# alexandervakhitov/lld-slam

Hardware: NVIDIA B200
Metric: local_ba_lm_iters_per_sec (higher is better)
Workload: dtype f64

## Files before the change

### lld_slam_b200/csrc/ba.cu

```cuda
#include <algorithm>
#include <atomic>
#include <chrono>
#include <condition_variable>
#include <functional>
#include <mutex>
#include <thread>
#include <cstdlib>
#include <cstring>
#ifdef __linux__
#include <sched.h>
#endif
#include <numeric>
#include <vector>

#include "ba_kernels.cuh"
#include "cr_solver.cuh"
#include "sp_solver.cuh"
#include "lld_ctx.h"

#include <array>
#include <map>
#include <string>

#ifdef LLD_WITH_NCCL
// ... 922 lines not shown
          spos[i] = oi;
          mask[oi] = (uint32_t)key[i];
          run += __builtin_popcountll(key[i]);
          w0[oi + 1] = run;
        }
      });
    };
    slots(p->pt_off, pt_order, pt_key, pt_spos, pts_mask, pts_w0, pl_off);
    slots(p->ln_off, ln_order, ln_key, ln_spos, lns_mask, lns_w0, ll_off);
    n_pw = (size_t)pts_w0[n_pt]; n_lw = (size_t)lns_w0[n_ln];
    stage("dense: W slots");
    int PIECE_CAP = 128;
    while (PIECE_CAP > 8 && (long long)(n_pt + n_ln) * 5 / (2 * PIECE_CAP) < 16LL * c->sm_count) PIECE_CAP >>= 1;
    using Job = BaDenseJob;
    auto& jobs = H.jobs;
    if (jobs.size() < 2 * (size_t)nw) jobs.resize(2 * (size_t)nw);
    for (size_t j = 0; j < 2 * (size_t)nw; j++) jobs[j].clear();
    const size_t n_jobs = 2 * (size_t)nw;
    par_for(2 * nw, [&](int jid) {
      const int kind = jid / nw, w = jid % nw;
      Job& J = jobs[jid];
      const int* loff = kind == 0 ? p->pt_off : p->ln_off;
      const pvec<uint32_t>& mask = kind == 0 ? pts_mask : lns_mask;
      const int g0 = w_g0[w];
      int b = loff[w];
      while (b < loff[w + 1]) {
        int e = b + 1;
        while (e < loff[w + 1] && mask[e] == mask[b] && e - b < PIECE_CAP) e++;
        const uint32_t m = mask[b];
        const int n = __builtin_popcount(m);
        if (n > 0) {
          const int pc = (int)J.pb.size();
          J.pb.push_back(b); J.pe.push_back(e); J.pn.push_back(n); J.pout.push_back(J.dsize);
          const int npair = n * (n + 1) / 2, ntask = 6 * npair + n;
          int hl[32], k = 0;
          for (int h = 0; h < 32; h++)
            if ((m >> h) & 1u) hl[k++] = h;
          int pr = 0;
          for (int ia = 0; ia < n; ia++)
            for (int ib = ia; ib < n; ib++, pr++) J.gb.push_back({nb_off[g0 + hl[ia]] + (hl[ib] - hl[ia]), J.dsize + 36LL * pr});
          for (int ia = 0; ia < n; ia++) J.gv.push_back({g0 + hl[ia], J.dsize + 36LL * npair + (long long)SCHUR_KS * ia});
          for (int t0 = 0; t0 < 2 * npair + n; t0 += SP_TPB) { J.itp.push_back(pc); J.itt.push_back(t0); }
          J.dsize += 36LL * npair + (long long)SCHUR_KS * n;
        }
        b = e;
      }
    });
    stage("dense: pieces");
    std::vector<long long> jd(n_jobs + 1, 0);
    std::vector<int> ji(n_jobs + 1, 0);
    for (size_t jid = 0; jid < n_jobs; jid++) {
      jd[jid + 1] = jd[jid] + jobs[jid].dsize;
      ji[jid + 1] = ji[jid] + (int)jobs[jid].itp.size();
    }
    dpart_total = jd[n_jobs];
    n_items_pt = ji[std::min<size_t>((size_t)nw, n_jobs)];
    n_items_all = ji[n_jobs];
    H.it_rec.resize(std::max(ji[n_jobs], 1));
    gb_off.assign(nb_g.size() + 1, 0);
    gv_off.assign(nG + 1, 0);
    par_for((int)n_jobs, [&](int jid) {
      Job& J = jobs[jid];
      const int ibase = ji[jid];
      const int kind = jid / nw, jw = jid % nw;
      for (size_t k = 0; k < J.itp.size(); k++) {
        const int q = J.itp[k];
        SchurItem& R = H.it_rec[ibase + k];
        R.l0 = J.pb[q]; R.nl = J.pe[q] - J.pb[q]; R.n = J.pn[q]; R.t0 = J.itt[k];
        R.w = jw; R.w0 = (kind == 0 ? pts_w0 : lns_w0)[J.pb[q]]; R.out = J.pout[q] + jd[jid];
        schur_item_shape(kind == 0 ? 3 : 4, R.n, R.nl, R.t0, &R.lc, &R.S, &R.nchunk);
      }
    });
    stage("dense: item records");
    {
      auto& tmp = H.it_tmp; auto& keys = H.it_keys;
      tmp.resize(H.it_rec.size()); keys.resize(H.it_rec.size());
      auto item_order = [&](int kind) {
        const int i0 = kind == 0 ? 0 : n_items_pt, i1 = kind == 0 ? n_items_pt : ji[n_jobs];
        const int cntk = i1 - i0;
        if (cntk <= 0) return;
        const int G = std::min(cntk, 4 * c->sm_count);
        constexpr int NB = 1024;
        std::vector<int> cnt(NB + 1, 0);
        for (int i = i0; i < i1; i++) {
          const SchurItem& R = H.it_rec[i];
          const int ntask = R.n * (R.n + 1) + R.n;
          const uint64_t cost = 64 + (uint64_t)R.nl * (uint64_t)(std::min(ntask - R.t0, (int)SP_TPB) + R.n + 1);
          const int bkt = NB - 1 - (int)std::min<uint64_t>(cost >> 5, NB - 1);
          keys[i] = (uint64_t)bkt;
          cnt[bkt + 1]++;
          tmp[i] = R;
        }
        for (int q = 0; q < NB; q++) cnt[q + 1] += cnt[q];
        for (int i = i0; i < i1; i++) {
          const int k = cnt[(int)keys[i]]++;
          const int r = k / G, j = k - r * G, len = std::min(G, cntk - r * G);
          const int pos = (r & 1) ? len - 1 - j : j;
          H.it_rec[i0 + r * G + pos] = tmp[i];
        }
      };
      par_for(nw + 2, [&](int t) {
        if (t < 2) { item_order(t); return; }
        const int w = t - 2;
        for (int kind = 0; kind < 2; kind++) {
          Job& J = jobs[(size_t)kind * nw + w];
          for (auto& x : J.gb) gb_off[x.first + 1]++;
          for (auto& x : J.gv) gv_off[x.first + 1]++;
        }
      });
    }
    stage("dense: item order + gather counts");
    for (size_t i = 0; i < nb_g.size(); i++) gb_off[i + 1] += gb_off[i];
    for (int i = 0; i < nG; i++) gv_off[i + 1] += gv_off[i];
    gb_src.resize(std::max<size_t>((size_t)gb_off[nb_g.size()], 1));
    gv_src.resize(std::max<size_t>((size_t)gv_off[nG], 1));
    {
      std::vector<int> curb(gb_off.begin(), gb_off.end() - 1), curv(gv_off.begin(), gv_off.end() - 1);
      par_for(nw, [&](int w) {
        for (int kind = 0; kind < 2; kind++) {
          const size_t jid = (size_t)kind * nw + w;
// ... 145 lines not shown
      return LLD_ERR_UNSUPPORTED;
    }
  }
  std::vector<long long> w_scr(nw, 0);
  long long scr_total = 0;
  for (int w = 0; w < nw; w++) {
    const long long n = 6LL * (w_g0[w + 1] - w_g0[w]);
    w_scr[w] = scr_total;
    if (S->max_n > SMEM_SOLVE_MAX_N && !v.env_mode) scr_total += n * n + 8 * n + 40;
  }

  stage("chunks");
  UP(tmp_i, kf_win.data(), n_kf); v.kf_win = tmp_i;
  int *d_pt_win, *d_ln_win, *d_pe_pt, *d_lc_ln, *d_pe_wpos, *d_lc_wpos;
  DEV(d_pt_win, int, n_pt); v.pt_win = d_pt_win;
  DEV(d_ln_win, int, n_ln); v.ln_win = d_ln_win;
  UP(tmp_i, kf_g.data(), n_kf); v.kf_g = tmp_i;
  UP(tmp_i, g_kf.data(), nG); v.g_kf = tmp_i;
  UP(tmp_i, w_g0.data(), nw + 1); v.w_g0 = tmp_i;
  DEV(d_pe_pt, int, n_pe); v.pe_pt = d_pe_pt;
  DEV(d_lc_ln, int, n_lc); v.lc_ln = d_lc_ln;
  UP(tmp_i, pe_pos.data(), dense ? 0 : n_pe); v.pe_pos = tmp_i;
  UP(tmp_i, lc_pos.data(), dense ? 0 : n_lc); v.lc_pos = tmp_i;
  UP(tmp_i, ch_g.data(), n_ch); v.ch_g = tmp_i;
  UP(tmp_i, ch_begin.data(), n_ch); v.ch_begin = tmp_i;
  UP(tmp_i, ch_end.data(), n_ch); v.ch_end = tmp_i;
  UP(tmp_i, ch_seg0.data(), ch_seg0.size()); v.ch_seg0 = tmp_i;
  UP(tmp_i, seg_begin.data(), seg_begin.size()); v.seg_begin = tmp_i;
  UP(tmp_i, seg_end.data(), seg_end.size()); v.seg_end = tmp_i;
  UP(tmp_i, g_chp0.data(), nG + 1); v.g_chp0 = tmp_i;
  UP(tmp_i, g_chl0.data(), nG + 1); v.g_chl0 = tmp_i;
  UP(tmp_i, nb_off.data(), nG + 1); v.nb_off = tmp_i;
  UP(tmp_i, nb_g.data(), nb_g.size()); v.nb_g = tmp_i;
  int *d_pl_tab = nullptr, *d_ll_tab = nullptr;
  DEV(d_pl_tab, int, std::max(pl_tab_total, 1LL)); v.pl_tab = d_pl_tab;
  DEV(d_ll_tab, int, std::max(ll_tab_total, 1LL)); v.ll_tab = d_ll_tab;
  long long* tmp_l;
  UP(tmp_l, pl_tab_off.data(), nG); v.pl_tab_off = tmp_l;
  UP(tmp_l, ll_tab_off.data(), nG); v.ll_tab_off = tmp_l;
  UP(tmp_l, ch_S_off.data(), n_ch); v.ch_S_off = tmp_l;
  UP(tmp_i, pt_spos.data(), n_pt); v.pt_spos = tmp_i;
  UP(tmp_i, ln_spos.data(), n_ln); v.ln_spos = tmp_i;
  UP(tmp_i, pts_w0.data(), n_pt + 1); v.pts_w0 = tmp_i;
  UP(tmp_i, lns_w0.data(), n_ln + 1); v.lns_w0 = tmp_i;
  DEV(d_pe_wpos, int, n_pe); v.pe_wpos = d_pe_wpos;
  DEV(d_lc_wpos, int, n_lc); v.lc_wpos = d_lc_wpos;
  { SchurItem* tmp_r; UP(tmp_r, H.it_rec.data(), (size_t)n_items_all); v.it_rec = tmp_r; }
  UP(tmp_i, gb_off.data(), gb_off.size()); v.gb_off = tmp_i;
  UP(tmp_l, gb_src.data(), gb_src.size()); v.gb_src = tmp_l;
  UP(tmp_i, gv_off.data(), gv_off.size()); v.gv_off = tmp_i;
  UP(tmp_l, gv_src.data(), gv_src.size()); v.gv_src = tmp_l;
  {
    uint32_t* tmp_m;
    UP(tmp_m, pts_mask.data(), n_pt); v.pts_mask = tmp_m;
    UP(tmp_m, lns_mask.data(), n_ln); v.lns_mask = tmp_m;
  }
  UP(tmp_l, w_scr.data(), nw); v.w_scratch_off = tmp_l;
  UP(tmp_i, env_first.data(), env_first.size()); v.env_first = tmp_i;
  UP(tmp_i, env_blk_last.data(), env_blk_last.size()); v.env_blk_last = tmp_i;
  UP(tmp_l, env_rowptr.data(), env_rowptr.size()); v.env_rowptr = tmp_l;

  stage("H2D enqueue");
  if (c->host_only) return LLD_OK;
  for (int b = 0; b < 2; b++) {
    DEV(v.pose_qt[b], double, 7 * (size_t)n_kf);
    DEV(v.pose_Rt[b], double, 12 * (size_t)n_kf);
// ... 67 lines not shown
    const bool dense_single = v.dense_mode && !(global_mode && c->n_ranks > 1) && v.n_slices == 1 && S->max_n <= SMEM_SOLVE_MAX_N && !v.env_mode;
    S->forked = allow && dense_single;
    S->use_graph = allow && dense_single;
    S->lean = dense_single;
  }
  {
    auto grid = [](int n) { return (n + 255) / 256; };
    if (n_pt) LLD_LAUNCH(c, k_expand_owner, grid(n_pt), 256, 0, n_pt, nw, v.pt_off, d_pt_win);
    if (n_ln) LLD_LAUNCH(c, k_expand_owner, grid(n_ln), 256, 0, n_ln, nw, v.ln_off, d_ln_win);
    if (n_pe) LLD_LAUNCH(c, k_expand_owner, grid(n_pe), 256, 0, n_pe, n_pt, v.pt_obs_off, d_pe_pt);
    if (n_lc) LLD_LAUNCH(c, k_expand_owner, grid(n_lc), 256, 0, n_lc, n_ln, v.ln_obs_off, d_lc_ln);
    if (!v.dense_mode) {
      LLD_CUDA(c, cudaMemsetAsync(d_pl_tab, 0xFF, sizeof(int) * (size_t)std::max(pl_tab_total, 1LL), c->stream));
      LLD_CUDA(c, cudaMemsetAsync(d_ll_tab, 0xFF, sizeof(int) * (size_t)std::max(ll_tab_total, 1LL), c->stream));
      if (n_plist) LLD_LAUNCH(c, k_build_tab, grid(n_plist), 256, 0, n_plist, nG, v.pl_off, v.pl_edge, v.pt_obs_off, v.pe_pt, v.pe_kf, v.kf_g,
                              v.pe_pos, v.nb_off, v.nb_g, v.pl_tab_off, d_pl_tab);
      if (n_llist) LLD_LAUNCH(c, k_build_tab, grid(n_llist), 256, 0, n_llist, nG, v.ll_off, v.ll_cell, v.ln_obs_off, v.lc_ln, v.lc_kf, v.kf_g,
                              v.lc_pos, v.nb_off, v.nb_g, v.ll_tab_off, d_ll_tab);
      if (tab_check) {
        std::vector<int> back((size_t)std::max(std::max(pl_tab_total, ll_tab_total), 1LL));
        for (int which = 0; which < 2; which++) {
          const long long tot = which ? ll_tab_total : pl_tab_total;
          LLD_CUDA(c, cudaMemcpyAsync(back.data(), which ? d_ll_tab : d_pl_tab, sizeof(int) * (size_t)tot, cudaMemcpyDeviceToHost, c->stream));
          LLD_CUDA(c, cudaStreamSynchronize(c->stream));
          const pvec<int>& ref = which ? ll_tab : pl_tab;
          long long bad = 0;
          for (long long k = 0; k < tot; k++) bad += back[(size_t)k] != ref[(size_t)k];
          fprintf(stderr, "[lld_ba_upload] LLD_TAB_CHECK %s table: %lld entries, %lld differ from the host build\n", which ? "line" : "point", tot, bad);
          if (bad) { snprintf(c->err, sizeof(c->err), "device-built position table differs from the host build"); return LLD_ERR_CUDA; }
        }
      }
    }
    if (v.dense_mode) {
      if (n_pe) LLD_LAUNCH(c, k_dense_wpos, grid(n_pe), 256, 0, n_pe, v.pe_pt, v.pe_kf, v.kf_g, v.pt_win, v.w_g0, v.pt_spos, v.pts_mask, v.pts_w0, d_pe_wpos);
      if (n_lc) LLD_LAUNCH(c, k_dense_wpos, grid(n_lc), 256, 0, n_lc, v.lc_ln, v.lc_kf, v.kf_g, v.ln_win, v.w_g0, v.ln_spos, v.lns_mask, v.lns_w0, d_lc_wpos);
    }
    LLD_CUDA(c, cudaGetLastError());
  }
  if (v.dense_mode) {
    LLD_CUDA(c, lld_raise_dyn_smem(k_schur_tile<3>, (size_t)SP_SMEM_BYTES));
    LLD_CUDA(c, lld_raise_dyn_smem(k_schur_tile<4>, (size_t)SP_SMEM_BYTES));
  }
  if (v.env_mode && S->use_cr) {
    LLD_CUDA(c, lld_raise_dyn_smem(k_cr_factor, sizeof(double) * ((size_t)S->cr.m * S->cr.m + 8 * (size_t)S->cr.m + 40)));
    LLD_CUDA(c, lld_raise_dyn_smem(k_cr_solve<15>, sizeof(double) * ((size_t)S->cr.m * S->cr.m + CR_RPT * CR_TC)));
    LLD_CUDA(c, lld_raise_dyn_smem(k_cr_solve<20>, sizeof(double) * ((size_t)S->cr.m * S->cr.m + CR_RPT * CR_TC)));
  } else if (v.env_mode && S->use_sp) {
    LLD_CUDA(c, lld_raise_dyn_smem(k_sp_factor, sizeof(double) * ((size_t)S->sp.m * S->sp.m + 8 * (size_t)S->sp.m + 40)));
    LLD_CUDA(c, lld_raise_dyn_smem(k_sp_solve<15>, sizeof(double) * ((size_t)S->sp.m * S->sp.m + CR_RPT * CR_TC)));
    LLD_CUDA(c, lld_raise_dyn_smem(k_sp_solve<20>, sizeof(double) * ((size_t)S->sp.m * S->sp.m + CR_RPT * CR_TC)));
  } else if (v.env_mode) LLD_CUDA(c, lld_raise_dyn_smem(k_solve_env, (size_t)(int)S->env_smem));
  else if (S->max_n <= SMEM_SOLVE_MAX_N)
    LLD_CUDA(c, lld_raise_dyn_smem(k_solve<true>, (size_t)(int)(sizeof(double) * ((size_t)S->max_n * S->max_n + 8 * (size_t)S->max_n + 40))));
  S->topo_ok = topo_cache && th != 0;
  return LLD_OK;
}

static inline int cdiv(int a, int b) { return (a + b - 1) / b; }

static int ba_init_state(LldCtx* c) {
  BaState* S = c->ba;
  BaView& v = S->v;
  const int n = std::max({v.n_kf, v.n_pt, v.n_ln, v.n_pe, v.n_lc, v.n_free_total, 1});
  LLD_LAUNCH(c, k_init_state, cdiv(n, 256), 256, 0, v, S->d_kf_Tcw_in, S->d_pt_in, S->d_ln_in, v.lc_right);
  LLD_CUDA(c, cudaGetLastError());
  return LLD_OK;
// ... 249 lines not shown
    if (r) return r;
  } else if (v.env_mode) {
    LLD_LAUNCH(c, k_solve_env, 1, 1024, S->env_smem, v);
  } else if (S->max_n <= SMEM_SOLVE_MAX_N) { int r = launch_solve<true>(c, v, S->max_n); if (r) return r; }
  else { int r = launch_solve<false>(c, v, S->max_n); if (r) return r; }
  if (par) LLD_CUDA(c, cudaEventRecord(c->ev_fork, s0));
  LLD_CUDA(c, fork(s1));
  if (v.n_pt && v.n_pt <= PT_WIDE_MAX) LLD_LAUNCH_S(c, s0, k_backsub_points<4>, cdiv(v.n_pt * 4, LM_TPB), LM_TPB, 0, v);
  else if (v.n_pt) LLD_LAUNCH_S(c, s0, k_backsub_points<1>, gp, LM_TPB, 0, v);
  { int r = launch_line_kernel(c, s1, v, false); if (r) return r; }
  LLD_CUDA(c, join(0));
  if (fused) {
    LLD_LAUNCH(c, k_decide_fused, v.n_win, FUSED_RED_TPB, 0, v, round, stop_now);
  } else {
    LLD_LAUNCH(c, k_reduce_trial, v.n_win * v.n_slices, 256, 0, v);
    LLD_LAUNCH(c, k_sum_trial, cdiv(v.n_win, 64), 64, 0, v);
    if (multi) { int r = ba_allreduce_trial(c); if (r) return r; }
    LLD_LAUNCH(c, k_decide, cdiv(v.n_win, 64), 64, 0, v, round, stop_now);
  }
  LLD_CUDA(c, cudaGetLastError());
  return LLD_OK;
}

static int ba_run_round(LldCtx* c, int maxit, int round, const volatile uint8_t* stop) {
  BaState* S = c->ba;
  BaView& v = S->v;
  LLD_LAUNCH(c, k_round_init, cdiv(v.n_win, 64), 64, 0, v, maxit, round);
  if (maxit <= 0) return LLD_OK;
  int* h_active = reinterpret_cast<int*>(c->pinned);
  const bool multi = S->global_mode && c->n_ranks > 1;
  const int hard_cap = maxit * 10 + 4;
  static const int group_len = getenv("LLD_BA_GROUP") ? std::max(1, atoi(getenv("LLD_BA_GROUP"))) : 2;
  int launched = 0;
  auto one_step = [&](int stop_now) -> int {
    const bool first = launched == 0;
    const int kind = (S->lean && !first) ? 1 : 0;
    if (S->use_graph && !c->prof_on && !stop_now && round < 2) {
      if (!S->graph_fresh[round][kind]) {
        const int64_t l0 = c->launches;
        cudaGraph_t g = nullptr;
        std::lock_guard<std::mutex> lk(lld_capture_mutex());
        LLD_CUDA(c, cudaStreamBeginCapture(c->stream, cudaStreamCaptureModeThreadLocal));
        int r = ba_step(c, round, 0, first);
        cudaError_t e = cudaStreamEndCapture(c->stream, &g);
        if (r) { if (g) cudaGraphDestroy(g); return r; }
        LLD_CUDA(c, e);
        bool updated = false;
        if (c->ba_graph[round][kind]) {
          cudaGraphExecUpdateResultInfo info;
          if (cudaGraphExecUpdate(c->ba_graph[round][kind], g, &info) == cudaSuccess) updated = true;
          else {
            cudaGetLastError();
            cudaGraphExecDestroy(c->ba_graph[round][kind]);
            c->ba_graph[round][kind] = nullptr;
          }
        }
        if (!updated) e = cudaGraphInstantiate(&c->ba_graph[round][kind], g, 0);
        cudaGraphDestroy(g);
        LLD_CUDA(c, e);
        c->ba_graph_kernels[round][kind] = (int)(c->launches - l0);
        c->launches = l0;
        S->graph_fresh[round][kind] = true;
      }
      {
        std::lock_guard<std::mutex> lk(lld_capture_mutex());
        LLD_CUDA(c, cudaGraphLaunch(c->ba_graph[round][kind], c->stream));
      }
      c->launches += c->ba_graph_kernels[round][kind];
      return LLD_OK;
    }
    return ba_step(c, round, stop_now, first);
  };
  for (int k = 0;; k++) {
    const int slot = k & 1;
    if (k >= 2) {
      LLD_CUDA(c, cudaEventSynchronize(c->ev_grp[slot]));
      if (h_active[slot] <= 0) break;
    }
    int stop_now = (stop && *stop) ? 1 : 0;
#ifdef LLD_WITH_NCCL
    if (multi && stop) {
      h_active[2] = stop_now;
      LLD_CUDA(c, cudaMemcpyAsync(v.n_active_win + 1, &h_active[2], sizeof(int), cudaMemcpyHostToDevice, c->stream));
      LLD_NCCL(c, ncclAllReduce(v.n_active_win + 1, v.n_active_win + 1, 1, ncclInt, ncclMax, reinterpret_cast<ncclComm_t>(c->comm), c->stream));
      LLD_CUDA(c, cudaMemcpyAsync(&h_active[2], v.n_active_win + 1, sizeof(int), cudaMemcpyDeviceToHost, c->stream));
      LLD_CUDA(c, cudaStreamSynchronize(c->stream));
      stop_now = h_active[2];
    }
#endif
    const int n = stop_now ? 1 : group_len;
    for (int s2 = 0; s2 < n; s2++) {
      int r = one_step(stop_now);
      if (r) return r;
      launched++;
    }
    LLD_CUDA(c, cudaMemcpyAsync(&h_active[slot], v.n_active_win, sizeof(int), cudaMemcpyDeviceToHost, c->stream));
    LLD_CUDA(c, cudaEventRecord(c->ev_grp[slot], c->stream));
    if (stop_now) break;
    if (launched >= hard_cap + 2 * group_len) {
      LLD_CUDA(c, cudaStreamSynchronize(c->stream));
      snprintf(c->err, sizeof(c->err), "LM step budget exhausted (%d steps, %d windows still active)", launched, h_active[slot]);
      return LLD_ERR_CUDA;
    }
  }
  LLD_CUDA(c, cudaStreamSynchronize(c->stream));
  return LLD_OK;
}

static int ba_download(LldCtx* c, const lld_ba_problem* p, lld_ba_result* out, bool local) {
  BaState* S = c->ba;
  BaView& v = S->v;
  const int n = std::max({v.n_kf, v.n_pt, v.n_ln, 1});
  if (local) {
    if (v.n_pe) LLD_LAUNCH(c, k_flag_points, cdiv(v.n_pe, 256), 256, 0, v, S->d_pt_bad);
    if (v.n_ln) LLD_LAUNCH(c, k_final_lines, cdiv(v.n_ln, 128), 128, 0, v, S->d_ln_bad);
  }
  LLD_LAUNCH(c, k_export, cdiv(n, 256), 256, 0, v, S->d_out_kf, S->d_out_pt, S->d_out_ln, S->d_ln_in);
  LLD_CUDA(c, cudaGetLastError());
  LLD_CUDA(c, cudaEventRecord(c->ev[2], c->stream));
  auto D2H = [&](void* dst, const void* src, size_t bytes) -> cudaError_t {
    if (!dst || !bytes) return cudaSuccess;
    return cudaMemcpyAsync(dst, src, bytes, cudaMemcpyDeviceToHost, c->stream);
  };
  LLD_CUDA(c, D2H(out->kf_Tcw, S->d_out_kf, sizeof(double) * 12 * (size_t)v.n_kf));
  LLD_CUDA(c, D2H(out->pt_xyz, S->d_out_pt, sizeof(double) * 3 * (size_t)v.n_pt));
  LLD_CUDA(c, D2H(out->ln_x0_dir, S->d_out_ln, sizeof(double) * 6 * (size_t)v.n_ln));
  LLD_CUDA(c, D2H(out->pt_obs_bad, S->d_pt_bad, (size_t)v.n_pe));
  LLD_CUDA(c, D2H(out->ln_obs_bad, S->d_ln_bad, 2 * (size_t)v.n_lc));
// ... 319 lines not shown
```

### lld_slam_b200/csrc/ba.cuh

```cuda
#pragma once
#include <stdint.h>

namespace lld {

enum : int { PH_LIN = 0, PH_RETRY = 1, PH_DONE = 2 };

constexpr int SCHUR_KS = 6;

struct BaParams {
  int robust_pt, robust_ln;
  double delta_pt_mono, delta_pt_stereo, delta_ln_mono, delta_ln_stereo;
  double chi2_pt_mono, chi2_pt_stereo;
  int ln_norm;
  int ln_filter;
};

struct __align__(16) SchurItem {
  int l0, nl, n, t0;
  int w, lc;
  long long w0;
  long long out;
  int S, nchunk;
};

struct BaView {
  int n_win, n_kf, n_pt, n_ln, n_pe, n_lc;
  int n_free_total;
  int n_chunks;
  const int *kf_off, *pt_off, *ln_off;
  const int *kf_win, *pt_win, *ln_win;
  const int* kf_g;
  const int* g_kf;
  const int* w_g0;
  const double* kf_intr;
  const double* kf_lcam;
  const int* pt_obs_off;
  const int* pe_kf;
  const int* pe_pt;
  const float* pe_uvr;
  const float* pe_info;
  const int* ln_obs_off;
  const int* lc_kf;
  const int* lc_ln;
  const float* lc_left;
  const float* lc_right;
  const double* lc_info;
  const uint8_t* lc_stereo;
  int n_chunks_pt;
  const int* pl_off;
  const int* pl_edge;
  const int* pe_pos;
  const int* ll_off;
  const int* ll_cell;
  const int* lc_pos;
  const int* ch_g;
  const int* ch_begin;
  const int* ch_end;
  const int* ch_seg0;
  const int* seg_begin;
  const int* seg_end;
  const int* g_chp0;
  const int* g_chl0;
  const int* nb_off;
  const int* nb_g;
  const int* pl_tab;
  const long long* pl_tab_off;
  const int* ll_tab;
  const long long* ll_tab_off;
  int n_fold, n_fold_pt;
  const int* fold_off;
  const int* fold_dst;
  const int* fold_src;
  int dense_mode;
  const int* pt_sorted;
  const int* ln_sorted;
  const int* pt_spos;
  const int* ln_spos;
  const uint32_t* pts_mask;
  const uint32_t* lns_mask;
  const int* pts_w0;
  const int* lns_w0;
  const int* pe_wpos;
  const int* lc_wpos;
  int n_items;
  int n_items_pt;
  const SchurItem* it_rec;
  const int* gb_off;
  const long long* gb_src;
  const int* gv_off;
  const long long* gv_src;
  double* pe_Wl;
  double* lc_Wl;
  double* pts_D;
  double* lns_D;
  double* dpart;
  double* pose_qt[2];
  double* pose_Rt[2];
// ... 66 lines not shown
```

### lld_slam_b200/csrc/ba_kernels.cuh

```cuda
#pragma once
#include <cfloat>
#include <cstdio>

#include "ba.cuh"
#include "lld_math.cuh"

namespace lld {

#define LM_TPB 128

__device__ __forceinline__ double warp_sum(double v) {
#pragma unroll
  for (int o = 16; o > 0; o >>= 1) v += __shfl_down_sync(0xffffffffu, v, o);
  return v;
}
__device__ __forceinline__ double warp_max(double v) {
#pragma unroll
  for (int o = 16; o > 0; o >>= 1) v = fmax(v, __shfl_down_sync(0xffffffffu, v, o));
  return v;
}
__device__ __forceinline__ double block_sum(double v, double* sm ) {
  const int lane = threadIdx.x & 31, wid = threadIdx.x >> 5;
  v = warp_sum(v);
  __syncthreads();
// ... 995 lines not shown
  const double lam = v.w_lambda[w];
  for (int t = threadIdx.x; t < ld; t += blockDim.x) {
    const int j = t / 6, c = t - 6 * j;
    double s[6] = {0, 0, 0, 0, 0, 0};
    double sb = 0;
    for (int rng = 0; rng < 2; rng++) {
      const int c0 = rng == 0 ? v.g_chp0[g] : v.g_chl0[g], c1 = rng == 0 ? v.g_chp0[g + 1] : v.g_chl0[g + 1];
      for (int ch = c0; ch < c1; ch++) {
        const double* part = v.ch_S + v.ch_S_off[ch];
#pragma unroll
        for (int r = 0; r < 6; r++) s[r] += part[(size_t)r * ld + t];
        if (j == 0) sb += part[(size_t)6 * ld + c];
      }
    }
    double* S = v.S_blk + 36 * (size_t)(v.nb_off[g] + j);
#pragma unroll
    for (int r = 0; r < 6; r++) {
      double d = 0.0;
      if (j == 0 && with_diag) {
        const int rr = r < c ? r : c, cc = r < c ? c : r;
        d = v.g_Hpp[21 * (size_t)g + (rr * 6 - (rr * (rr - 1)) / 2 + (cc - rr))];
        if (r == c) d += lam;
      }
      S[6 * r + c] = d - s[r];
    }
    if (j == 0) v.g_bs[6 * (size_t)g + c] = (with_diag ? v.g_bp[6 * (size_t)g + c] : 0.0) - sb;
  }
}

constexpr int SP_TPB = 128;
constexpr int SP_CAP_WD = 2304;
constexpr int SP_CAP_Z = 2560;
constexpr int SP_SMEM_BYTES = (2 * SP_CAP_WD + SP_CAP_Z) * 8;
constexpr int SP_MAX_S = 16;

__device__ __forceinline__ void cp_async16(void* dst_smem, const void* src) {
  const unsigned s = (unsigned)__cvta_generic_to_shared(dst_smem);
  asm volatile("cp.async.cg.shared.global [%0], [%1], 16;\n" ::"r"(s), "l"(src));
}

inline void schur_item_shape(int D, int n, int nl, int t0, int* lc, int* S, int* nchunk) {
  const int WS = 6 * D, DS = D == 3 ? 10 : 14;
  const int ntask = n * (n + 1) + n;
  int ntb = ntask - t0 < SP_TPB ? ntask - t0 : SP_TPB;
  if (ntb < 1) ntb = 1;
  int L = SP_CAP_WD / (n * WS + DS);
  const int Lz = SP_CAP_Z / ((n + 1) * WS);
  if (Lz < L) L = Lz;
  if (nl < L) L = nl;
  int s = SP_TPB / ntb;
  if (s > SP_MAX_S) s = SP_MAX_S;
  if (s > L / 2) s = L / 2;
  if (s < 1) s = 1;
  *lc = L; *S = s; *nchunk = (nl + L - 1) / L;
}

template <int D>
__global__ void __launch_bounds__(SP_TPB, 4) k_schur_tile(BaView v, int item_base, int n_items) {
  constexpr int WS = 6 * D;
  constexpr int DS = D == 3 ? 10 : 14;
  constexpr int OFF_C = D * (D + 1) / 2;
  extern __shared__ __align__(16) double sp_smem[];
  double* const sZ = sp_smem + 2 * SP_CAP_WD;
  const int tid = threadIdx.x, lane = tid & 31;
  const int G = gridDim.x;
  const int cnt = (n_items - (int)blockIdx.x + G - 1) / G;
  const SchurItem* items = v.it_rec + item_base + blockIdx.x;
  const double* Wbase = D == 3 ? v.pe_Wl : v.lc_Wl;
  const double* Dbase = D == 3 ? v.pts_D : v.lns_D;

  int scan_base = -32;
  unsigned scan_mask = 0;
  auto next_item = [&]() -> int {
    while (true) {
      if (scan_mask) {
        const int j = __ffs(scan_mask) - 1;
        scan_mask &= scan_mask - 1;
        return scan_base + j;
      }
      scan_base += 32;
      if (scan_base >= cnt) return -1;
      const int j = scan_base + lane;
      bool a = false;
      if (j < cnt) a = v.w_phase[items[(size_t)j * G].w] != PH_DONE;
      scan_mask = __ballot_sync(0xffffffffu, a);
    }
  };
  auto load_item = [&](int k, SchurItem& R) {
    const int4* p = reinterpret_cast<const int4*>(items + (size_t)k * G);
    const int4 a = p[0], b = p[1];
    R.l0 = a.x; R.nl = a.y; R.n = a.z; R.t0 = a.w;
    R.w = b.x;
    R.w0 = ((long long)(unsigned)b.w << 32) | (unsigned)b.z;
    const int4 c2 = p[2];
    R.out = ((long long)(unsigned)c2.y << 32) | (unsigned)c2.x;
    R.lc = b.y; R.S = c2.z; R.nchunk = c2.w;
  };
  auto issue = [&](const SchurItem& R, int c, int b) {
    const int rowW = R.n * WS;
    const int Lc = R.lc;
    const int lc0 = c * Lc, m = min(Lc, R.nl - lc0);
    double* sW = sp_smem + b * SP_CAP_WD;
    double* sD = sW + Lc * rowW;
    const double* gW = Wbase + (size_t)R.w0 * WS + (size_t)lc0 * rowW;
    const int nW = m * rowW / 2;
    for (int i = tid; i < nW; i += SP_TPB) cp_async16(sW + 2 * i, gW + 2 * i);
    const double* gD = Dbase + (size_t)(R.l0 + lc0) * DS;
    const int nD = m * DS / 2;
    for (int i = tid; i < nD; i += SP_TPB) cp_async16(sD + 2 * i, gD + 2 * i);
  };

  int cur = next_item();
  if (cur < 0) return;
  SchurItem R, Rn;
  load_item(cur, R);
  issue(R, 0, 0);
  asm volatile("cp.async.commit_group;\n" ::);
  int nxt = next_item();
  Rn = R;
  if (nxt >= 0) load_item(nxt, Rn);
  int buf = 0, c = 0;
  while (true) {
    const int n = R.n, nl = R.nl;
    const int npair = n * (n + 1) / 2, ntask = 2 * npair + n;
    const int ntb = min(SP_TPB, ntask - R.t0);
    const int rowW = n * WS, rowZ = (n + 1) * WS;
    const int Lc = R.lc, nchunk = R.nchunk, S = R.S;
    const int s = tid / ntb, tl = tid - s * ntb;
    const bool act = s < S;
    int ia = 0, zb = n, h = 0;
    {
      const int task = R.t0 + tl;
      if (task < 2 * npair) {
        int pr = task >> 1;
        h = task & 1;
        while (pr >= n - ia) { pr -= n - ia; ia++; }
        zb = ia + pr;
      } else {
        ia = min(task - 2 * npair, n - 1);
      }
    }
    const int zl0 = tid / (n + 1), zb0 = tid - zl0 * (n + 1);
    const int zdl = SP_TPB / (n + 1), zdb = SP_TPB - zdl * (n + 1);
    double acc[18];
#pragma unroll
    for (int q = 0; q < 18; q++) acc[q] = 0.0;
    for (c = 0; c < nchunk; c++, buf ^= 1) {
      if (c + 1 < nchunk) issue(R, c + 1, buf ^ 1);
      else if (nxt >= 0) issue(Rn, 0, buf ^ 1);
      asm volatile("cp.async.commit_group;\n" ::);
      asm volatile("cp.async.wait_group 1;\n" ::: "memory");
      __syncthreads();
      const int m = min(Lc, nl - c * Lc);
      const double* sW = sp_smem + buf * SP_CAP_WD;
      const double* sD = sW + Lc * rowW;
      for (int i = tid, l = zl0, b = zb0; i < m * (n + 1); i += SP_TPB) {
        const double* Dv = sD + l * DS;
        double* z = sZ + l * rowZ + b * WS;
        if (b < n) {
          const double* wv = sW + l * rowW + b * WS;
          double dm[D][D];
#pragma unroll
          for (int k = 0; k < D; k++)
#pragma unroll
            for (int j = 0; j < D; j++) {
              const int r = k < j ? k : j, c2 = k < j ? j : k;
              dm[k][j] = Dv[r * D - (r * (r - 1)) / 2 + (c2 - r)];
            }
#pragma unroll
          for (int cc = 0; cc < 6; cc++) {
            double wb[D];
#pragma unroll
            for (int j = 0; j < D; j++) wb[j] = wv[cc * D + j];
#pragma unroll
            for (int k = 0; k < D; k++) {
              double zz = 0;
#pragma unroll
              for (int j = 0; j < D; j++) zz += dm[k][j] * wb[j];
              z[cc * D + k] = zz;
            }
          }
        } else {
#pragma unroll
          for (int k = 0; k < WS; k++) z[k] = k < D ? Dv[OFF_C + k] : 0.0;
        }
        l += zdl; b += zdb;
        if (b > n) { b -= n + 1; l++; }
      }
      __syncthreads();
      if (act) {
        const double* wa_p = sW + ia * WS;
        const double* z_p = sZ + zb * WS + h * 3 * D;
#pragma unroll 2
        for (int l = s; l < m; l += S) {
          double wa[WS];
          const double* wp = wa_p + l * rowW;
#pragma unroll
          for (int k = 0; k < WS; k += 2) {
            const double2 t2 = *reinterpret_cast<const double2*>(wp + k);
            wa[k] = t2.x; wa[k + 1] = t2.y;
          }
          const double* zp = z_p + l * rowZ;
#pragma unroll
          for (int cc = 0; cc < 3; cc++) {
            double z[D];
#pragma unroll
            for (int k = 0; k < D; k++) z[k] = zp[cc * D + k];
#pragma unroll
            for (int r = 0; r < 6; r++) {
              double a2 = acc[cc * 6 + r];
#pragma unroll
              for (int k = 0; k < D; k++) a2 += wa[D * r + k] * z[k];
              acc[cc * 6 + r] = a2;
            }
          }
        }
      }
      __syncthreads();
    }
    double* out = v.dpart + R.out;
    if (S == 1) {
      if (tid < ntb) {
        const int task = R.t0 + tl;
        if (task < 2 * npair) {
          double* o = out + (size_t)(task >> 1) * 36 + (task & 1) * 18;
#pragma unroll
          for (int q = 0; q < 18; q++) o[q] = acc[q];
        } else {
          double* o = out + (size_t)36 * npair + (size_t)(task - 2 * npair) * SCHUR_KS;
#pragma unroll
          for (int q = 0; q < 6; q++) o[q] = acc[q];
        }
      }
    } else {
      double* red = sZ;
      if (act)
#pragma unroll
        for (int q = 0; q < 18; q++) red[(s * ntb + tl) * 18 + q] = acc[q];
      __syncthreads();
      for (int e = tid; e < ntb * 18; e += SP_TPB) {
        const int tl2 = e / 18, q = e - 18 * tl2;
        const int task = R.t0 + tl2;
        size_t o;
        if (task < 2 * npair) o = (size_t)(task >> 1) * 36 + (task & 1) * 18 + q;
        else if (q < 6) o = (size_t)36 * npair + (size_t)(task - 2 * npair) * SCHUR_KS + q;
        else continue;
        double sum = 0;
        for (int s2 = 0; s2 < S; s2++) sum += red[(s2 * ntb + tl2) * 18 + q];
        out[o] = sum;
      }
    }
    if (nxt < 0) break;
    cur = nxt;
    R = Rn;
    nxt = next_item();
    if (nxt >= 0) load_item(nxt, Rn);
  }
}

__global__ void __launch_bounds__(256) k_reduce_piece(BaView v, int n_blocks) {
  const int t = blockIdx.x * blockDim.x + threadIdx.x;
  if (t < n_blocks * 36) {
    const int blk = t / 36, e = t - 36 * blk, c = e / 6, r = e - 6 * c;
    int lo = 0, hi = v.n_free_total;
    while (hi - lo > 1) {
      const int mid = (lo + hi) >> 1;
      if (v.nb_off[mid] <= blk) lo = mid;
      else hi = mid;
    }
    const int g = lo, j = blk - v.nb_off[g];
    const int w = v.kf_win[v.g_kf[g]];
    if (v.w_phase[w] == PH_DONE) return;
    double s = 0;
    const int q1 = v.gb_off[blk + 1];
    int q = v.gb_off[blk];
    for (; q + 8 <= q1; q += 8) {
      long long o[8];
      double a[8];
#pragma unroll
      for (int k = 0; k < 8; k++) o[k] = v.gb_src[q + k];
#pragma unroll
      for (int k = 0; k < 8; k++) a[k] = v.dpart[o[k] + e];
#pragma unroll
      for (int k = 0; k < 8; k++) s += a[k];
    }
    for (; q + 4 <= q1; q += 4) {
      const long long o0 = v.gb_src[q], o1 = v.gb_src[q + 1], o2 = v.gb_src[q + 2], o3 = v.gb_src[q + 3];
      const double a0 = v.dpart[o0 + e], a1 = v.dpart[o1 + e], a2 = v.dpart[o2 + e], a3 = v.dpart[o3 + e];
      s += a0; s += a1; s += a2; s += a3;
    }
    for (; q < q1; q++) s += v.dpart[v.gb_src[q] + e];
    double d = 0.0;
    if (j == 0) {
      const int rr = r < c ? r : c, cc = r < c ? c : r;
      d = v.g_Hpp[21 * (size_t)g + (rr * 6 - (rr * (rr - 1)) / 2 + (cc - rr))];
      if (r == c) d += v.w_lambda[w];
    }
    v.S_blk[36 * (size_t)blk + 6 * r + c] = d - s;
  } else {
    const int u = t - n_blocks * 36;
    const int g = u / 6, r = u - 6 * g;
    if (g >= v.n_free_total) return;
    const int w = v.kf_win[v.g_kf[g]];
    if (v.w_phase[w] == PH_DONE) return;
    double s = 0;
    for (int q = v.gv_off[g]; q < v.gv_off[g + 1]; q++) s += v.dpart[v.gv_src[q] + r];
    v.g_bs[6 * (size_t)g + r] = v.g_bp[6 * (size_t)g + r] - s;
  }
}

__global__ void __launch_bounds__(256) k_reduce_piece_warp(BaView v, int n_blocks) {
  const int wi = blockIdx.x * (blockDim.x >> 5) + (threadIdx.x >> 5);
  const int lane = threadIdx.x & 31;
  if (wi < n_blocks * 6) {
    const int blk = wi / 6, c = wi - 6 * blk;
    int lo = 0, hi = v.n_free_total;
    while (hi - lo > 1) {
      const int mid = (lo + hi) >> 1;
      if (v.nb_off[mid] <= blk) lo = mid;
      else hi = mid;
    }
    const int g = lo, j = blk - v.nb_off[g];
    const int w = v.kf_win[v.g_kf[g]];
    if (v.w_phase[w] == PH_DONE) return;
    double s[6] = {0, 0, 0, 0, 0, 0};
    for (int q = v.gb_off[blk] + lane; q < v.gb_off[blk + 1]; q += 32) {
      const double* src = v.dpart + v.gb_src[q] + 6 * c;
#pragma unroll
      for (int r = 0; r < 6; r++) s[r] += src[r];
    }
#pragma unroll
    for (int r = 0; r < 6; r++) s[r] = warp_sum(s[r]);
    if (lane == 0) {
      const double lam = v.w_lambda[w];
#pragma unroll
      for (int r = 0; r < 6; r++) {
        double d = 0.0;
        if (j == 0) {
          const int rr = r < c ? r : c, cc = r < c ? c : r;
          d = v.g_Hpp[21 * (size_t)g + (rr * 6 - (rr * (rr - 1)) / 2 + (cc - rr))];
          if (r == c) d += lam;
        }
        v.S_blk[36 * (size_t)blk + 6 * r + c] = d - s[r];
      }
    }
  } else {
    const int g = wi - n_blocks * 6;
    if (g >= v.n_free_total) return;
    const int w = v.kf_win[v.g_kf[g]];
    if (v.w_phase[w] == PH_DONE) return;
    double s[6] = {0, 0, 0, 0, 0, 0};
    for (int q = v.gv_off[g] + lane; q < v.gv_off[g + 1]; q += 32) {
      const double* src = v.dpart + v.gv_src[q];
#pragma unroll
      for (int r = 0; r < 6; r++) s[r] += src[r];
    }
#pragma unroll
    for (int r = 0; r < 6; r++) s[r] = warp_sum(s[r]);
    if (lane == 0)
#pragma unroll
      for (int r = 0; r < 6; r++) v.g_bs[6 * (size_t)g + r] = v.g_bp[6 * (size_t)g + r] - s[r];
  }
}

__device__ __forceinline__ double rcp_newton(double d) {
  double r;
  asm("rcp.approx.ftz.f64 %0, %1;" : "=d"(r) : "d"(d));
  double e = fma(-d, r, 1.0);
  r = fma(r, e, r);
  e = fma(-d, r, 1.0);
  r = fma(r, e, r);
  return r;
}

__device__ bool ldlt_solve_cta(double* __restrict__ A, int n, int ld, double* __restrict__ b , double* __restrict__ tmp, int* flag) {
  const int tid = threadIdx.x, nt = blockDim.x;
  const int lane = tid & 31, wid = tid >> 5, nw = nt >> 5;
  double* Tt = tmp;
  double* zb = tmp + 6 * n;
  int li = 0, lj = lane;
  while (li < 5 && lj > li) { lj -= li + 1; li++; }
  auto factor = [&](int k0, double* zq) -> bool {
// ... 962 lines not shown
```

Baseline: 79250.

## Compute dense Schur piece blocks with FP64 mma.sync 8x8x4 tiles

Replaces the per-thread scalar FMA accumulation of 6x6 Schur blocks with warp-level FP64 tensor core mma.sync m8n8k4 over 8x8 tiles of the upper-triangular piece matrix, each warp owning up to four tiles. Item splitting and cost estimation now count tiles instead of tasks, and the cross-slice shared-memory reduction is removed. Outputs are scattered from mma fragments into the packed block layout, including mirroring diagonal blocks. The trade-off is padding waste on partial tiles and strided shared-memory fragment loads.

```diff
diff --git a/lld_slam_b200/csrc/ba.cu b/lld_slam_b200/csrc/ba.cu
--- a/lld_slam_b200/csrc/ba.cu
+++ b/lld_slam_b200/csrc/ba.cu
@@ -978,7 +978,7 @@
         if (n > 0) {
           const int pc = (int)J.pb.size();
           J.pb.push_back(b); J.pe.push_back(e); J.pn.push_back(n); J.pout.push_back(J.dsize);
-          const int npair = n * (n + 1) / 2, ntask = 6 * npair + n;
+          const int npair = n * (n + 1) / 2;
           int hl[32], k = 0;
           for (int h = 0; h < 32; h++)
             if ((m >> h) & 1u) hl[k++] = h;
@@ -986,7 +986,7 @@
           for (int ia = 0; ia < n; ia++)
             for (int ib = ia; ib < n; ib++, pr++) J.gb.push_back({nb_off[g0 + hl[ia]] + (hl[ib] - hl[ia]), J.dsize + 36LL * pr});
           for (int ia = 0; ia < n; ia++) J.gv.push_back({g0 + hl[ia], J.dsize + 36LL * npair + (long long)SCHUR_KS * ia});
-          for (int t0 = 0; t0 < 2 * npair + n; t0 += SP_TPB) { J.itp.push_back(pc); J.itt.push_back(t0); }
+          for (int t0 = 0, nt = schur_piece_tiles(n); t0 < nt; t0 += SP_TILES) { J.itp.push_back(pc); J.itt.push_back(t0); }
           J.dsize += 36LL * npair + (long long)SCHUR_KS * n;
         }
         b = e;
@@ -1014,7 +1014,7 @@
         SchurItem& R = H.it_rec[ibase + k];
         R.l0 = J.pb[q]; R.nl = J.pe[q] - J.pb[q]; R.n = J.pn[q]; R.t0 = J.itt[k];
         R.w = jw; R.w0 = (kind == 0 ? pts_w0 : lns_w0)[J.pb[q]]; R.out = J.pout[q] + jd[jid];
-        schur_item_shape(kind == 0 ? 3 : 4, R.n, R.nl, R.t0, &R.lc, &R.S, &R.nchunk);
+        schur_item_shape(kind == 0 ? 3 : 4, R.n, R.nl, R.t0, &R.lc, &R.nt, &R.nchunk);
       }
     });
     stage("dense: item records");
@@ -1030,8 +1030,7 @@
         std::vector<int> cnt(NB + 1, 0);
         for (int i = i0; i < i1; i++) {
           const SchurItem& R = H.it_rec[i];
-          const int ntask = R.n * (R.n + 1) + R.n;
-          const uint64_t cost = 64 + (uint64_t)R.nl * (uint64_t)(std::min(ntask - R.t0, (int)SP_TPB) + R.n + 1);
+          const uint64_t cost = 64 + (uint64_t)R.nl * (uint64_t)(2 * R.nt + R.n + 1);
           const int bkt = NB - 1 - (int)std::min<uint64_t>(cost >> 5, NB - 1);
           keys[i] = (uint64_t)bkt;
           cnt[bkt + 1]++;
diff --git a/lld_slam_b200/csrc/ba.cuh b/lld_slam_b200/csrc/ba.cuh
--- a/lld_slam_b200/csrc/ba.cuh
+++ b/lld_slam_b200/csrc/ba.cuh
@@ -20,7 +20,7 @@
   int w, lc;
   long long w0;
   long long out;
-  int S, nchunk;
+  int nt, nchunk;
 };
 
 struct BaView {
diff --git a/lld_slam_b200/csrc/ba_kernels.cuh b/lld_slam_b200/csrc/ba_kernels.cuh
--- a/lld_slam_b200/csrc/ba_kernels.cuh
+++ b/lld_slam_b200/csrc/ba_kernels.cuh
@@ -1051,27 +1051,32 @@
 constexpr int SP_CAP_WD = 2304;
 constexpr int SP_CAP_Z = 2560;
 constexpr int SP_SMEM_BYTES = (2 * SP_CAP_WD + SP_CAP_Z) * 8;
-constexpr int SP_MAX_S = 16;
+constexpr int SP_TW = 4;
+constexpr int SP_TILES = SP_TW * SP_TPB / 32;
 
 __device__ __forceinline__ void cp_async16(void* dst_smem, const void* src) {
   const unsigned s = (unsigned)__cvta_generic_to_shared(dst_smem);
   asm volatile("cp.async.cg.shared.global [%0], [%1], 16;\n" ::"r"(s), "l"(src));
 }
 
-inline void schur_item_shape(int D, int n, int nl, int t0, int* lc, int* S, int* nchunk) {
+__device__ __forceinline__ void dmma_884(double (&c)[2], double a, double b) {
+  asm("mma.sync.aligned.m8n8k4.row.col.f64.f64.f64.f64 {%0, %1}, {%2}, {%3}, {%0, %1};\n"
+      : "+d"(c[0]), "+d"(c[1]) : "d"(a), "d"(b));
+}
+
+inline int schur_piece_tiles(int n) {
+  const int Tr = (6 * n + 7) / 8, Tc = (6 * n + 8) / 8;
+  return Tr * Tc - Tr * (Tr - 1) / 2;
+}
+
+inline void schur_item_shape(int D, int n, int nl, int t0, int* lc, int* nt, int* nchunk) {
   const int WS = 6 * D, DS = D == 3 ? 10 : 14;
-  const int ntask = n * (n + 1) + n;
-  int ntb = ntask - t0 < SP_TPB ? ntask - t0 : SP_TPB;
-  if (ntb < 1) ntb = 1;
+  const int rest = schur_piece_tiles(n) - t0;
   int L = SP_CAP_WD / (n * WS + DS);
   const int Lz = SP_CAP_Z / ((n + 1) * WS);
   if (Lz < L) L = Lz;
   if (nl < L) L = nl;
-  int s = SP_TPB / ntb;
-  if (s > SP_MAX_S) s = SP_MAX_S;
-  if (s > L / 2) s = L / 2;
-  if (s < 1) s = 1;
-  *lc = L; *S = s; *nchunk = (nl + L - 1) / L;
+  *lc = L; *nt = rest < SP_TILES ? rest : SP_TILES; *nchunk = (nl + L - 1) / L;
 }
 
 template <int D>
@@ -1113,7 +1118,7 @@
     R.w0 = ((long long)(unsigned)b.w << 32) | (unsigned)b.z;
     const int4 c2 = p[2];
     R.out = ((long long)(unsigned)c2.y << 32) | (unsigned)c2.x;
-    R.lc = b.y; R.S = c2.z; R.nchunk = c2.w;
+    R.lc = b.y; R.nt = c2.z; R.nchunk = c2.w;
   };
   auto issue = [&](const SchurItem& R, int c, int b) {
     const int rowW = R.n * WS;
@@ -1141,29 +1146,29 @@
   int buf = 0, c = 0;
   while (true) {
     const int n = R.n, nl = R.nl;
-    const int npair = n * (n + 1) / 2, ntask = 2 * npair + n;
-    const int ntb = min(SP_TPB, ntask - R.t0);
     const int rowW = n * WS, rowZ = (n + 1) * WS;
-    const int Lc = R.lc, nchunk = R.nchunk, S = R.S;
-    const int s = tid / ntb, tl = tid - s * ntb;
-    const bool act = s < S;
-    int ia = 0, zb = n, h = 0;
+    const int Lc = R.lc, nchunk = R.nchunk;
+    const int Tc = (6 * n + 8) >> 3;
+    const int wid = tid >> 5, g = lane >> 2, q = lane & 3;
+    const int mynt = R.nt > wid ? (R.nt - wid + 3) >> 2 : 0;
+    int ti[SP_TW], tj[SP_TW];
     {
-      const int task = R.t0 + tl;
-      if (task < 2 * npair) {
-        int pr = task >> 1;
-        h = task & 1;
-        while (pr >= n - ia) { pr -= n - ia; ia++; }
-        zb = ia + pr;
-      } else {
-        ia = min(task - 2 * npair, n - 1);
+      int i = 0, j = mynt ? R.t0 + wid : 0;
+      while (j >= Tc - i) { j -= Tc - i; i++; }
+      j += i;
+#pragma unroll
+      for (int k = 0; k < SP_TW; k++) {
+        ti[k] = i; tj[k] = j;
+#pragma unroll
+        for (int u = 0; u < 4; u++)
+          if (++j == Tc) { i++; j = i; }
       }
     }
     const int zl0 = tid / (n + 1), zb0 = tid - zl0 * (n + 1);
     const int zdl = SP_TPB / (n + 1), zdb = SP_TPB - zdl * (n + 1);
-    double acc[18];
-#pragma unroll
-    for (int q = 0; q < 18; q++) acc[q] = 0.0;
+    double acc[SP_TW][2];
+#pragma unroll
+    for (int k = 0; k < SP_TW; k++) acc[k][0] = acc[k][1] = 0.0;
     for (c = 0; c < nchunk; c++, buf ^= 1) {
       if (c + 1 < nchunk) issue(R, c + 1, buf ^ 1);
       else if (nxt >= 0) issue(Rn, 0, buf ^ 1);
@@ -1207,30 +1212,21 @@
         if (b > n) { b -= n + 1; l++; }
       }
       __syncthreads();
-      if (act) {
-        const double* wa_p = sW + ia * WS;
-        const double* z_p = sZ + zb * WS + h * 3 * D;
-#pragma unroll 2
-        for (int l = s; l < m; l += S) {
-          double wa[WS];
-          const double* wp = wa_p + l * rowW;
-#pragma unroll
-          for (int k = 0; k < WS; k += 2) {
-            const double2 t2 = *reinterpret_cast<const double2*>(wp + k);
-            wa[k] = t2.x; wa[k + 1] = t2.y;
-          }
-          const double* zp = z_p + l * rowZ;
-#pragma unroll
-          for (int cc = 0; cc < 3; cc++) {
-            double z[D];
-#pragma unroll
-            for (int k = 0; k < D; k++) z[k] = zp[cc * D + k];
-#pragma unroll
-            for (int r = 0; r < 6; r++) {
-              double a2 = acc[cc * 6 + r];
-#pragma unroll
-              for (int k = 0; k < D; k++) a2 += wa[D * r + k] * z[k];
-              acc[cc * 6 + r] = a2;
+      {
+        const int K = D * m;
+        for (int k0 = 0; k0 < K; k0 += 4) {
+          const int kk = k0 + q;
+          const bool valid = kk < K;
+          const int l = valid ? kk / D : 0, d = valid ? kk - l * D : 0;
+          const double* pA = sW + l * rowW + d;
+          const double* pB = sZ + l * rowZ + d;
+#pragma unroll
+          for (int k = 0; k < SP_TW; k++) {
+            if (k < mynt) {
+              const int r = 8 * ti[k] + g, cb = 8 * tj[k] + g;
+              const double a = (valid && r < 6 * n) ? pA[r * D] : 0.0;
+              const double b = cb < 6 * n + 6 ? pB[cb * D] : 0.0;
+              dmma_884(acc[k], a, b);
             }
           }
         }
@@ -1238,35 +1234,23 @@
       __syncthreads();
     }
     double* out = v.dpart + R.out;
-    if (S == 1) {
-      if (tid < ntb) {
-        const int task = R.t0 + tl;
-        if (task < 2 * npair) {
-          double* o = out + (size_t)(task >> 1) * 36 + (task & 1) * 18;
-#pragma unroll
-          for (int q = 0; q < 18; q++) o[q] = acc[q];
-        } else {
-          double* o = out + (size_t)36 * npair + (size_t)(task - 2 * npair) * SCHUR_KS;
-#pragma unroll
-          for (int q = 0; q < 6; q++) o[q] = acc[q];
+    const int npair = n * (n + 1) / 2;
+#pragma unroll
+    for (int k = 0; k < SP_TW; k++) {
+      if (k < mynt) {
+        const int Rr = 8 * ti[k] + g;
+#pragma unroll
+        for (int e = 0; e < 2; e++) {
+          const int C = 8 * tj[k] + 2 * q + e;
+          if (Rr >= 6 * n || C > 6 * n) continue;
+          const int a = Rr / 6, r = Rr - 6 * a;
+          if (C == 6 * n) { out[36 * (size_t)npair + SCHUR_KS * a + r] = acc[k][e]; continue; }
+          const int b = C / 6, c2 = C - 6 * b;
+          if (a > b || (a == b && r > c2)) continue;
+          double* o = out + 36 * (size_t)(a * n - a * (a - 1) / 2 + b - a);
+          o[6 * c2 + r] = acc[k][e];
+          if (a == b && r < c2) o[6 * r + c2] = acc[k][e];
         }
-      }
-    } else {
-      double* red = sZ;
-      if (act)
-#pragma unroll
-        for (int q = 0; q < 18; q++) red[(s * ntb + tl) * 18 + q] = acc[q];
-      __syncthreads();
-      for (int e = tid; e < ntb * 18; e += SP_TPB) {
-        const int tl2 = e / 18, q = e - 18 * tl2;
-        const int task = R.t0 + tl2;
-        size_t o;
-        if (task < 2 * npair) o = (size_t)(task >> 1) * 36 + (task & 1) * 18 + q;
-        else if (q < 6) o = (size_t)36 * npair + (size_t)(task - 2 * npair) * SCHUR_KS + q;
-        else continue;
-        double sum = 0;
-        for (int s2 = 0; s2 < S; s2++) sum += red[(s2 * ntb + tl2) * 18 + q];
-        out[o] = sum;
       }
     }
     if (nxt < 0) break;
```

After: 74020 (median of 6 runs). -6.6%, worse.

## Capture grouped LM steps in one graph and precompute block owner tables

Applied to the files above, without the earlier changes.

Graph capture now records a whole group of LM steps (group_len, default two) in a single CUDA graph instead of one step per graph, which halves graph launches per host sync. The graph kind is now always 1 after the first step rather than depending on the lean flag. In the reduce kernels, the per-thread binary search over nb_off and the kf_win[g_kf[g]] double indirection are replaced by lookup tables (blk_g, g_win) filled once at upload by a k_expand_owner kernel. The tables are only allocated in dense mode, so the reduce kernels would read null pointers if they run outside dense mode. The kernel is used but not defined in the lines shown.

```diff
diff --git a/lld_slam_b200/csrc/ba.cu b/lld_slam_b200/csrc/ba.cu
--- a/lld_slam_b200/csrc/ba.cu
+++ b/lld_slam_b200/csrc/ba.cu
@@ -1243,6 +1243,9 @@
   UP(tmp_i, g_chl0.data(), nG + 1); v.g_chl0 = tmp_i;
   UP(tmp_i, nb_off.data(), nG + 1); v.nb_off = tmp_i;
   UP(tmp_i, nb_g.data(), nb_g.size()); v.nb_g = tmp_i;
+  int *d_blk_g, *d_g_win;
+  DEV(d_blk_g, int, dense ? nb_g.size() : 0); v.blk_g = d_blk_g;
+  DEV(d_g_win, int, dense ? nG : 0); v.g_win = d_g_win;
   int *d_pl_tab = nullptr, *d_ll_tab = nullptr;
   DEV(d_pl_tab, int, std::max(pl_tab_total, 1LL)); v.pl_tab = d_pl_tab;
   DEV(d_ll_tab, int, std::max(ll_tab_total, 1LL)); v.ll_tab = d_ll_tab;
@@ -1376,6 +1379,9 @@
       }
     }
     if (v.dense_mode) {
+      const int n_blk = (int)nb_g.size();
+      if (n_blk) LLD_LAUNCH(c, k_expand_owner, grid(n_blk), 256, 0, n_blk, nG, v.nb_off, d_blk_g);
+      if (nG) LLD_LAUNCH(c, k_expand_owner, grid(nG), 256, 0, nG, nw, v.w_g0, d_g_win);
       if (n_pe) LLD_LAUNCH(c, k_dense_wpos, grid(n_pe), 256, 0, n_pe, v.pe_pt, v.pe_kf, v.kf_g, v.pt_win, v.w_g0, v.pt_spos, v.pts_mask, v.pts_w0, d_pe_wpos);
       if (n_lc) LLD_LAUNCH(c, k_dense_wpos, grid(n_lc), 256, 0, n_lc, v.lc_ln, v.lc_kf, v.kf_g, v.ln_win, v.w_g0, v.ln_spos, v.lns_mask, v.lns_w0, d_lc_wpos);
     }
@@ -1691,16 +1697,17 @@
   const int hard_cap = maxit * 10 + 4;
   static const int group_len = getenv("LLD_BA_GROUP") ? std::max(1, atoi(getenv("LLD_BA_GROUP"))) : 2;
   int launched = 0;
-  auto one_step = [&](int stop_now) -> int {
+  auto one_group = [&](int n, int stop_now) -> int {
     const bool first = launched == 0;
-    const int kind = (S->lean && !first) ? 1 : 0;
+    const int kind = first ? 0 : 1;
     if (S->use_graph && !c->prof_on && !stop_now && round < 2) {
       if (!S->graph_fresh[round][kind]) {
         const int64_t l0 = c->launches;
         cudaGraph_t g = nullptr;
         std::lock_guard<std::mutex> lk(lld_capture_mutex());
         LLD_CUDA(c, cudaStreamBeginCapture(c->stream, cudaStreamCaptureModeThreadLocal));
-        int r = ba_step(c, round, 0, first);
+        int r = LLD_OK;
+        for (int s2 = 0; s2 < n && !r; s2++) r = ba_step(c, round, 0, first && s2 == 0);
         cudaError_t e = cudaStreamEndCapture(c->stream, &g);
         if (r) { if (g) cudaGraphDestroy(g); return r; }
         LLD_CUDA(c, e);
@@ -1728,7 +1735,11 @@
       c->launches += c->ba_graph_kernels[round][kind];
       return LLD_OK;
     }
-    return ba_step(c, round, stop_now, first);
+    for (int s2 = 0; s2 < n; s2++) {
+      int r = ba_step(c, round, stop_now, first && s2 == 0);
+      if (r) return r;
+    }
+    return LLD_OK;
   };
   for (int k = 0;; k++) {
     const int slot = k & 1;
@@ -1748,11 +1759,8 @@
     }
 #endif
     const int n = stop_now ? 1 : group_len;
-    for (int s2 = 0; s2 < n; s2++) {
-      int r = one_step(stop_now);
-      if (r) return r;
-      launched++;
-    }
+    { int r = one_group(n, stop_now); if (r) return r; }
+    launched += n;
     LLD_CUDA(c, cudaMemcpyAsync(&h_active[slot], v.n_active_win, sizeof(int), cudaMemcpyDeviceToHost, c->stream));
     LLD_CUDA(c, cudaEventRecord(c->ev_grp[slot], c->stream));
     if (stop_now) break;
diff --git a/lld_slam_b200/csrc/ba.cuh b/lld_slam_b200/csrc/ba.cuh
--- a/lld_slam_b200/csrc/ba.cuh
+++ b/lld_slam_b200/csrc/ba.cuh
@@ -63,6 +63,8 @@
   const int* g_chl0;
   const int* nb_off;
   const int* nb_g;
+  const int* blk_g;
+  const int* g_win;
   const int* pl_tab;
   const long long* pl_tab_off;
   const int* ll_tab;
diff --git a/lld_slam_b200/csrc/ba_kernels.cuh b/lld_slam_b200/csrc/ba_kernels.cuh
--- a/lld_slam_b200/csrc/ba_kernels.cuh
+++ b/lld_slam_b200/csrc/ba_kernels.cuh
@@ -1281,14 +1281,8 @@
   const int t = blockIdx.x * blockDim.x + threadIdx.x;
   if (t < n_blocks * 36) {
     const int blk = t / 36, e = t - 36 * blk, c = e / 6, r = e - 6 * c;
-    int lo = 0, hi = v.n_free_total;
-    while (hi - lo > 1) {
-      const int mid = (lo + hi) >> 1;
-      if (v.nb_off[mid] <= blk) lo = mid;
-      else hi = mid;
-    }
-    const int g = lo, j = blk - v.nb_off[g];
-    const int w = v.kf_win[v.g_kf[g]];
+    const int g = v.blk_g[blk], j = blk - v.nb_off[g];
+    const int w = v.g_win[g];
     if (v.w_phase[w] == PH_DONE) return;
     double s = 0;
     const int q1 = v.gb_off[blk + 1];
@@ -1320,7 +1314,7 @@
     const int u = t - n_blocks * 36;
     const int g = u / 6, r = u - 6 * g;
     if (g >= v.n_free_total) return;
-    const int w = v.kf_win[v.g_kf[g]];
+    const int w = v.g_win[g];
     if (v.w_phase[w] == PH_DONE) return;
     double s = 0;
     for (int q = v.gv_off[g]; q < v.gv_off[g + 1]; q++) s += v.dpart[v.gv_src[q] + r];
@@ -1333,14 +1327,8 @@
   const int lane = threadIdx.x & 31;
   if (wi < n_blocks * 6) {
     const int blk = wi / 6, c = wi - 6 * blk;
-    int lo = 0, hi = v.n_free_total;
-    while (hi - lo > 1) {
-      const int mid = (lo + hi) >> 1;
-      if (v.nb_off[mid] <= blk) lo = mid;
-      else hi = mid;
-    }
-    const int g = lo, j = blk - v.nb_off[g];
-    const int w = v.kf_win[v.g_kf[g]];
+    const int g = v.blk_g[blk], j = blk - v.nb_off[g];
+    const int w = v.g_win[g];
     if (v.w_phase[w] == PH_DONE) return;
     double s[6] = {0, 0, 0, 0, 0, 0};
     for (int q = v.gb_off[blk] + lane; q < v.gb_off[blk + 1]; q += 32) {
@@ -1366,7 +1354,7 @@
   } else {
     const int g = wi - n_blocks * 6;
     if (g >= v.n_free_total) return;
-    const int w = v.kf_win[v.g_kf[g]];
+    const int w = v.g_win[g];
     if (v.w_phase[w] == PH_DONE) return;
     double s[6] = {0, 0, 0, 0, 0, 0};
     for (int q = v.gv_off[g] + lane; q < v.gv_off[g + 1]; q += 32) {
```

Measured after the change: 79860 before, 80500 after, median of 6. About the same (+0.8%).
